# ezwelty/glimpse

Measured on NVIDIA B200. Metric: particle_updates_per_s, higher is better.
Workload: dtype f64

## Files before the change

### glimpse_b200/_lib.py

```python
from __future__ import annotations

import ctypes as C
import os

HERE = os.path.dirname(os.path.abspath(__file__))
LIB_PATH = os.path.join(HERE, "libglimpse_b200.so")

GB_MAX_OBS = 8
GB_ST_MESSAGES = {
    1: (ValueError, "Some particles are on non-visible viewshed cells"),
    2: (ValueError, "Some particles have missing (NaN) values"),
    3: (ValueError, "Some of the sampling coordinates are out of bounds"),
    4: (ValueError, "Some sampling points are outside box"),
    5: (IndexError, "Box extends beyond grid bounds"),
    6: (MemoryError, "Search window larger than the launch plan's surface capacity (template + 191 px per axis in mode='stream'; "
                     "the particle cloud has dispersed)"),
}
GB_OBS_OUT_OF_FRAME = 2
GB_ST_WINDOW_TOO_LARGE = 6
GB_WINDOW_MARGIN, GB_WINDOW_MARGIN_MAX = 191, 1000
GB_RNG_SUPPLIED, GB_RNG_PHILOX = 0, 1
GB_DRAW_WORDS, GB_DRAW_NORMALS, GB_DRAW_UNIFORM, GB_DRAW_UNIFORM_PARTICLE = 0, 1, 2, 3
GB_RESAMPLE = {"systematic": 0, "stratified": 1, "choice": 2, "residual": 3}
GB_MODE_STREAM = 1
# ... 77 lines not shown
        ("force_evolved", C.c_void_p), ("force_weights", C.c_void_p), ("dump_evolved", C.c_void_p),
        ("dump_uv", C.c_void_p), ("dump_box", C.c_void_p), ("dump_search", C.c_void_p), ("dump_sse", C.c_void_p),
        ("dump_sampled", C.c_void_p), ("dump_weights", C.c_void_p), ("dump_indices", C.c_void_p), ("dump_clocks", C.c_void_p), ("dump_cap", C.c_int64),
    ]


STRUCTS = (gb_camera, gb_image, gb_surface, gb_motion, gb_plan, gb_track_desc, gb_stage_io)

SIGNATURES = {
    "gb_version": (C.c_int, []),
    "gb_last_error": (C.c_char_p, []),
    "gb_struct_size": (C.c_int64, [C.c_int32]),
    "gb_sample_surface": (C.c_int, [C.c_void_p, C.c_int32, C.c_int32, C.c_int32, C.c_int32, C.c_void_p, C.c_int64, C.c_void_p, C.c_void_p, C.c_void_p]),
    "gb_kernel_timing": (C.c_int, [C.c_int32]),
    "gb_kernel_timing_read": (C.c_int, [C.POINTER(C.c_double), C.POINTER(C.c_int64), C.c_int32]),
    "gb_camera_from_vector": (C.c_int, [C.c_void_p, C.c_void_p, C.POINTER(gb_camera)]),
    "gb_project": (C.c_int, [C.POINTER(gb_camera), C.c_void_p, C.c_int64, C.c_void_p, C.c_void_p]),
    "gb_project_image": (C.c_int, [C.POINTER(gb_image), C.POINTER(gb_camera), C.c_int32, C.c_void_p, C.c_void_p]),
    "gb_viewshed_work_bytes": (C.c_int64, [C.c_int32, C.c_int32, C.c_int32]),
    "gb_viewshed": (C.c_int, [C.c_void_p, C.c_int32, C.c_int32, C.c_void_p, C.c_void_p, C.c_double, C.POINTER(C.c_double),
                              C.POINTER(C.c_double), C.c_int32, C.c_void_p, C.c_int64, C.c_void_p, C.c_void_p]),
    "gb_jpeg_info": (C.c_int, [C.c_char_p, C.c_int64, C.POINTER(C.c_int32), C.POINTER(C.c_int32), C.POINTER(C.c_int32)]),
    "gb_decode_jpeg": (C.c_int, [C.c_char_p, C.c_int64, C.c_int32, C.c_int32, C.c_int32, C.c_void_p, C.c_void_p]),
    "gb_unproject": (C.c_int, [C.POINTER(gb_camera), C.c_void_p, C.c_int64, C.c_int, C.c_void_p, C.c_void_p, C.c_void_p]),
    "gb_state_from_rows": (C.c_int, [C.c_void_p, C.c_int64, C.c_int64, C.c_void_p, C.c_void_p]),
    "gb_state_to_rows": (C.c_int, [C.c_void_p, C.c_int64, C.c_int64, C.c_void_p, C.c_void_p]),
    "gb_step_plan": (C.c_int, [C.c_int64, C.c_int32, C.c_int32, C.c_int64, C.c_int32, C.c_int32, C.c_int32, C.POINTER(gb_plan)]),
    "gb_step_plan_ex": (C.c_int, [C.c_int64, C.c_int32, C.c_int32, C.c_int64, C.c_int32, C.c_int32, C.c_int32, C.c_int32, C.POINTER(gb_plan)]),
    "gb_track": (C.c_int, [C.POINTER(gb_track_desc), C.c_void_p, C.POINTER(C.c_int64)]),
    "gb_track_step": (C.c_int, [C.POINTER(gb_track_desc), C.c_int32, C.POINTER(gb_stage_io), C.c_void_p]),
# ... 45 lines not shown
```

### glimpse_b200/csrc/camera.cuh

```cuda
#pragma once
#include "common.cuh"

namespace gb {

__device__ __forceinline__ void distort(const gb_camera& c, double x, double y, double& xd, double& yd) {
  const bool any_k = (c.k[0] != 0.0) | (c.k[1] != 0.0) | (c.k[2] != 0.0) | (c.k[3] != 0.0) | (c.k[4] != 0.0) |
                     (c.k[5] != 0.0);
  const bool any_p = (c.p[0] != 0.0) | (c.p[1] != 0.0);
  xd = x;
  yd = y;
  if (!any_k && !any_p) return;
  const double r2 = add(mul(x, x), mul(y, y));
  if (any_k) {
    double dr = 1.0;
    if (c.k[0] != 0.0) dr = add(dr, mul(c.k[0], r2));
    if (c.k[1] != 0.0) dr = add(dr, mul(mul(c.k[1], r2), r2));
    if (c.k[2] != 0.0) dr = add(dr, mul(mul(mul(c.k[2], r2), r2), r2));
    if ((c.k[3] != 0.0) | (c.k[4] != 0.0) | (c.k[5] != 0.0)) {
      double den = 1.0;
      if (c.k[3] != 0.0) den = add(den, mul(c.k[3], r2));
      if (c.k[4] != 0.0) den = add(den, mul(mul(c.k[4], r2), r2));
      if (c.k[5] != 0.0) den = add(den, mul(mul(mul(c.k[5], r2), r2), r2));
      dr = quo(dr, den);
    }
// ... 44 lines not shown
}

struct CamK {
  gb_camera c;
  int32_t any_k, any_p, has_den, pad_;
};

__host__ inline void camk_from(const gb_camera& c, CamK& out) {
  out.c = c;
  out.any_k = (c.k[0] != 0.0) || (c.k[1] != 0.0) || (c.k[2] != 0.0) || (c.k[3] != 0.0) || (c.k[4] != 0.0) || (c.k[5] != 0.0);
  out.has_den = (c.k[3] != 0.0) || (c.k[4] != 0.0) || (c.k[5] != 0.0);
  out.any_p = (c.p[0] != 0.0) || (c.p[1] != 0.0);
  out.pad_ = 0;
}

__device__ __forceinline__ void project_fast(const CamK& k, double px, double py, double pz, double& u, double& v) {
  const gb_camera& c = k.c;
  const double dx = px - c.xyz[0], dy = py - c.xyz[1];
  if (c.affine) {
    u = dx / c.f[0];
    v = dy / c.f[1];
    return;
  }
  double dz = pz - c.xyz[2];
  if (c.has_corr) dz = add(dz, quo(mul(c.corr_c1, add(mul(dx, dx), mul(dy, dy))), c.corr_c2));
  const double xc = fma(c.R[2], dz, fma(c.R[1], dy, c.R[0] * dx));
  const double yc = fma(c.R[5], dz, fma(c.R[4], dy, c.R[3] * dx));
  const double zc = fma(c.R[8], dz, fma(c.R[7], dy, c.R[6] * dx));
  double xd, yd;
  if (!k.any_k && !k.any_p) {
    const double iz = 1.0 / zc;
    xd = xc * iz;
    yd = yc * iz;
  } else {
    const double z2 = zc * zc, s = fma(xc, xc, yc * yc);
    const double s2 = s * s, z4 = z2 * z2;
    const double s3 = s2 * s, z6 = z4 * z2;
    const double sz4 = s * z4, s2z2 = s2 * z2;
    const double Nn = fma(c.k[2], s3, fma(c.k[1], s2z2, fma(c.k[0], sz4, z6)));
    const double Dd = k.has_den ? fma(c.k[5], s3, fma(c.k[4], s2z2, fma(c.k[3], sz4, z6))) : z6;
// ... 98 lines not shown
```

### glimpse_b200/csrc/glimpse_b200.cu

```cuda
#include <cuda.h>
#include <cuda_runtime.h>
#include <dlfcn.h>
#include <math.h>
#include <nvjpeg.h>
#include <stdio.h>
#include <stdlib.h>
#include <string.h>

#include <mutex>
#include <vector>

#include "camera.cuh"
#include "common.cuh"
#include "motion.cuh"
#include "tile.cuh"

#define GB_THREADS 512
#define GB_MAX_TEMPLATE 1024
#define GB_MAX_HIGHPASS 31

namespace gb {

static thread_local char g_error[512] = "";

// ... 75 lines not shown
  int64_t surf_bytes;
  int s_block, s_nblk;
  int tmpl_from_ev;
  int resample_method;
  int s2_budget;
  int s2_smem;
  int64_t p0, pb;
  int interp_rows, interp_cols;
};

struct NextParams {
  double tau, tau2;
  int spec_update, pad_;
  int img[GB_MAX_OBS];
  CamK cam[GB_MAX_OBS];
};

struct alignas(64) FrameMaps {
  CUtensorMap map[GB_MAX_OBS];
  int ok[GB_MAX_OBS];
};

__device__ __forceinline__ double* state_buffer(const StepParams& prm, int t) { return (t & 1) ? prm.state_b : prm.state_a; }

__device__ __forceinline__ int status_from_flags(uint32_t f) {
  if (f & GB_F_EVOLVE_OOB) return GB_ST_DEM_BOUNDS;
  if (f & GB_F_VIEW_OOB) return GB_ST_DEM_BOUNDS;
  if (f & GB_F_NOT_VISIBLE) return GB_ST_NOT_VISIBLE;
  if (f & GB_F_NAN) return GB_ST_NAN;
  if (f & GB_F_TEMPLATE) return GB_ST_TEMPLATE_BOUNDS;
  if (f & GB_F_WINDOW) return GB_ST_WINDOW_TOO_LARGE;
  if (f & GB_F_SAMPLE_OUTSIDE) return GB_ST_SAMPLE_OUTSIDE;
  if (f & GB_F_DEM_OOB) return GB_ST_DEM_BOUNDS;
  return GB_ST_OK;
}

__device__ __forceinline__ uint32_t test_particle(const StepParams& prm, const double (&s)[6]) {
  uint32_t f = 0;
  if (prm.viewshed >= 0) {
    bool oob;
    const double vis = surface_sample(prm.surfaces[prm.viewshed], s[0], s[1], 0, oob);
    if (oob) f |= GB_F_VIEW_OOB;
    else if (vis == 0.0) f |= GB_F_NOT_VISIBLE;
  }
  if (isnan(s[0]) | isnan(s[1]) | isnan(s[2]) | isnan(s[3]) | isnan(s[4]) | isnan(s[5])) f |= GB_F_NAN;
  return f;
}

template <bool COV>
struct Moments {
  static constexpr int NM = COV ? 28 : 13;
  double a[NM];
  __device__ __forceinline__ void clear() {
#pragma unroll
// ... 1002 lines not shown
    cudaEventRecord(next(), s);
  }
  void collect() {
    for (size_t i = 0; i < kind.size(); ++i) {
      float t = 0.f;
      if (cudaEventElapsedTime(&t, ev[2 * i], ev[2 * i + 1]) == cudaSuccess) {
        ms[kind[i]] += t;
        n[kind[i]] += 1;
      }
    }
    kind.clear();
    used = 0;
  }
};
static KernelTimer g_ktimer;

static int track_streaming(const gb_track_desc& d, cudaStream_t stream, int64_t* launches) {
  static std::once_flag attr_once[16];
  int dev = 0;
  GB_CUDA(cudaGetDevice(&dev));
  cudaError_t aerr = cudaSuccess;
  std::call_once(attr_once[dev & 15], [&]() {
    aerr = cudaFuncSetAttribute(k_s2_surface<false>, cudaFuncAttributeMaxDynamicSharedMemorySize, kSurfaceSmem);
    if (aerr == cudaSuccess) aerr = cudaFuncSetAttribute(k_s2_surface<true>, cudaFuncAttributeMaxDynamicSharedMemorySize, kSurfaceSmemLarge);
    if (aerr == cudaSuccess) aerr = cudaFuncSetAttribute(k_s4p_resample_propagate<true, true>, cudaFuncAttributeMaxDynamicSharedMemorySize, kS4pSmem);
    if (aerr == cudaSuccess) aerr = cudaFuncSetAttribute(k_s4p_resample_propagate<false, true>, cudaFuncAttributeMaxDynamicSharedMemorySize, kS4pSmem);
    if (aerr == cudaSuccess) aerr = cudaFuncSetAttribute(k_s4p_resample_propagate<true, false>, cudaFuncAttributeMaxDynamicSharedMemorySize, kS4pSmem);
    if (aerr == cudaSuccess) aerr = cudaFuncSetAttribute(k_s4p_resample_propagate<false, false>, cudaFuncAttributeMaxDynamicSharedMemorySize, kS4pSmem);
  });
  if (aerr != cudaSuccess) return fail(GB_E_CUDA, "stream kernel attributes: %s", cudaGetErrorString(aerr));
  if (d.plan.stream_block > GB_S4P_CAP || (d.plan.stream_block & 1)) return fail(GB_E_INVALID, "plan: stream_block must be even and <= 768%s");
  if (d.plan.stream_batch > 65535) return fail(GB_E_INVALID, "plan: stream_batch must be <= 65535%s");
  const bool cov = d.covariances != nullptr;
  const bool tangent = d.motion_kinds == 0 || (d.motion_kinds & ((1 << GB_MOTION_TANGENT_CARTESIAN) | (1 << GB_MOTION_TANGENT_CYLINDRICAL))) != 0;
  const int slots = d.plan.stream_slots;
  const int64_t batch = d.plan.stream_batch;
  const int64_t nbatch = (d.P + batch - 1) / batch;
  const int used = (int)(nbatch < slots ? nbatch : slots);
  StreamPool* pool = nullptr;
  int rc = get_pool(&pool);
  if (rc) return rc;
  std::lock_guard<std::mutex> guard(pool->busy);
  StepParams probe;
// ... 46 lines not shown
    if (launches) ++*launches;
  }
  bool have_activity = false;
  for (int t = 0; t < T; ++t) {
    if (!has_init[t] && !has_update[t] && !has_prop[t]) {
      have_activity = false;
      continue;
    }
    StepParams prm;
    fill_params(d, t, prm);
    NextParams nxt;
    memset(&nxt, 0, sizeof(nxt));
    for (int o = 0; o < GB_MAX_OBS; ++o) nxt.img[o] = -1;
    nxt.spec_update = has_init[t] ? 0 : 1;
    if (const char* e = getenv("GB_S4P_SPEC")) nxt.spec_update = nxt.spec_update && atoi(e) != 0;
    if (t + 1 < T) {
      StepParams pn;
      fill_params(d, t + 1, pn);
      nxt.tau = pn.tau;
      nxt.tau2 = pn.tau2;
      for (int o = 0; o < d.O; ++o) {
        nxt.img[o] = pn.img[o];
        nxt.cam[o] = pn.cam[o];
      }
    }
    FrameMaps fm;
    frame_maps(prm, fm);
    if (has_init[t] || has_tmpl[t]) {
      if ((rc = join_sides())) return rc;
      if ((rc = wait_images(stream, prm))) return rc;
      stream_bind(d, prm, t, 0, d.P);
      prm.tmpl_from_ev = 1;
      if (has_init[t]) {
        g_ktimer.begin(GB_K_INIT, stream);
        if ((rc = launch_init(prm, cov, stream))) return rc;
        g_ktimer.end(stream);
        if (launches) ++*launches;
      }
      if (has_tmpl[t]) {
        g_ktimer.begin(GB_K_TEMPLATE, stream);
// ... 31 lines not shown
          k_s2_surface<false><<<(unsigned)(pb * prm.O), GB_S2_THREADS, prm.s2_smem, ss>>>(prm, fm, prm.s2_budget);
        kt.end(ss);
        kt.begin(GB_K_WEIGHTS, ss);
        if (spline_is_hermite(prm.interp_cols, prm.interp_rows))
          k_s3_weights<false><<<dim3((unsigned)prm.s_nblk, (unsigned)pb), s3_threads(prm.s_block), 0, ss>>>(prm);
        else
          k_s3_weights<true><<<dim3((unsigned)prm.s_nblk, (unsigned)pb), s3_threads(prm.s_block), 0, ss>>>(prm);
        kt.end(ss);
        kt.begin(GB_K_PUBLISH, ss);
        k_s3b_publish<<<(unsigned)((pb + 7) / 8), 256, 0, ss>>>(prm);
        kt.end(ss);
      }
      kt.begin(GB_K_RESAMPLE_PROPAGATE, ss);
      {
        const dim3 grid((unsigned)prm.s_nblk, (unsigned)pb);
        if (cov && tangent)
          k_s4p_resample_propagate<true, true><<<grid, GB_S4P_THREADS, kS4pSmem, ss>>>(prm, nxt);
        else if (cov)
          k_s4p_resample_propagate<true, false><<<grid, GB_S4P_THREADS, kS4pSmem, ss>>>(prm, nxt);
        else if (tangent)
          k_s4p_resample_propagate<false, true><<<grid, GB_S4P_THREADS, kS4pSmem, ss>>>(prm, nxt);
        else
          k_s4p_resample_propagate<false, false><<<grid, GB_S4P_THREADS, kS4pSmem, ss>>>(prm, nxt);
      }
      kt.end(ss);
      kt.begin(GB_K_FINALIZE, ss);
      if (cov)
        k_s5p_finalize<true><<<(unsigned)((pb + 3) / 4), 128, 0, ss>>>(prm);
      else
        k_s5p_finalize<false><<<(unsigned)((pb + 3) / 4), 128, 0, ss>>>(prm);
      kt.end(ss);
      GB_CUDA(cudaGetLastError());
      if (launches) *launches += (has_update[t] ? 5 : 2) + (need_activity ? 1 : 0);
    }
  }
  if ((rc = join_sides())) return rc;
  if (g_ktimer.on) {
    GB_CUDA(cudaStreamSynchronize(stream));
// ... 118 lines not shown
    case 5: return sizeof(gb_track_desc);
    case 6: return sizeof(gb_stage_io);
    default: return -1;
  }
}

int gb_kernel_timing(int32_t enable) {
  std::lock_guard<std::mutex> guard(gb::g_ktimer.mu);
  gb::g_ktimer.on = enable != 0;
  gb::g_ktimer.kind.clear();
  gb::g_ktimer.used = 0;
  for (int k = 0; k < gb::GB_K_KINDS; ++k) {
    gb::g_ktimer.ms[k] = 0.0;
    gb::g_ktimer.n[k] = 0;
  }
  return GB_OK;
}

int gb_kernel_timing_read(double* ms, int64_t* launches, int32_t n) {
  if (!ms || !launches || n < 0) return gb::fail(GB_E_INVALID, "null argument%s");
  std::lock_guard<std::mutex> guard(gb::g_ktimer.mu);
  for (int k = 0; k < n; ++k) {
    ms[k] = k < gb::GB_K_KINDS ? gb::g_ktimer.ms[k] : 0.0;
    launches[k] = k < gb::GB_K_KINDS ? gb::g_ktimer.n[k] : 0;
  }
  return GB_OK;
}

int gb_camera_from_vector(const double* v, const double* corr, gb_camera* out) {
  if (!v || !out) return fail(GB_E_INVALID, "null argument%s");
// ... 434 lines not shown
```

### glimpse_b200/csrc/motion.cuh

```cuda
#pragma once
#include "common.cuh"

namespace gb {

struct Philox {
  uint32_t key0, key1;
  __device__ __forceinline__ static void round(uint32_t (&c)[4], uint32_t k0, uint32_t k1) {
    const uint32_t hi0 = __umulhi(0xD2511F53u, c[0]), lo0 = 0xD2511F53u * c[0];
    const uint32_t hi1 = __umulhi(0xCD9E8D57u, c[2]), lo1 = 0xCD9E8D57u * c[2];
    const uint32_t n0 = hi1 ^ c[1] ^ k0, n2 = hi0 ^ c[3] ^ k1;
    c[0] = n0;
    c[1] = lo1;
    c[2] = n2;
    c[3] = lo0;
  }
  __device__ __forceinline__ void generate(uint32_t c0, uint32_t c1, uint32_t c2, uint32_t c3, uint32_t (&out)[4]) const {
    uint32_t c[4] = {c0, c1, c2, c3};
    uint32_t k0 = key0, k1 = key1;
#pragma unroll
    for (int i = 0; i < 10; ++i) {
      round(c, k0, k1);
      k0 += 0x9E3779B9u;
      k1 += 0xBB67AE85u;
    }
    out[0] = c[0];
    out[1] = c[1];
    out[2] = c[2];
    out[3] = c[3];
  }
};

__device__ __forceinline__ void philox_normals3(uint64_t seed, uint64_t point, uint32_t time, uint32_t particle,
                                                uint32_t stream, double& z0, double& z1, double& z2, int need = 3) {
  Philox g{(uint32_t)seed, (uint32_t)(seed >> 32)};
  uint32_t r[4];
  g.generate(particle, time, (uint32_t)point, ((uint32_t)(point >> 32) << 8) | stream, r);
  const float two_neg32 = 2.3283064365386963e-10f;
  z0 = z1 = z2 = 0.0;
  if (need & 1) {
    const float u0 = ((float)r[0] + 0.5f) * two_neg32;
    const float a0 = fminf(fmaxf(u0, 1.0e-10f), 1.0f);
    const float e0 = fmaxf(-2.0f * __logf(a0), 1.0e-30f);
    const float rad0 = e0 * rsqrtf(e0);
    float s0, c0;
    __sincosf(6.283185307179586f * ((float)(r[1] >> 8) * 5.9604644775390625e-08f), &s0, &c0);
    z0 = (double)(rad0 * c0);
    z1 = (double)(rad0 * s0);
  }
  if (need & 2) {
    const float u1 = ((float)r[2] + 0.5f) * two_neg32;
    const float a1 = fminf(fmaxf(u1, 1.0e-10f), 1.0f);
    const float e1 = fmaxf(-2.0f * __logf(a1), 1.0e-30f);
    const float rad1 = e1 * rsqrtf(e1);
    z2 = (double)(rad1 * __cosf(6.283185307179586f * ((float)(r[3] >> 8) * 5.9604644775390625e-08f)));
  }
}

__device__ __forceinline__ bool motion_is_tangent(const gb_motion& m) { return m.kind >= GB_MOTION_TANGENT_CARTESIAN; }
__device__ __forceinline__ bool motion_is_cylindrical(const gb_motion& m) {
  return m.kind == GB_MOTION_CYLINDRICAL || m.kind == GB_MOTION_TANGENT_CYLINDRICAL;
}

__device__ __forceinline__ int evolve_needs(const gb_motion& m) {
  const double third = motion_is_tangent(m) ? m.slope_sigma : m.a_sigma[2];
  return ((m.a_sigma[0] != 0.0 || m.a_sigma[1] != 0.0) ? 1 : 0) | (third != 0.0 ? 2 : 0);
}

__device__ __forceinline__ double philox_uniform(uint64_t seed, uint64_t point, uint32_t time) {
  Philox g{(uint32_t)seed, (uint32_t)(seed >> 32)};
// ... 108 lines not shown
```

### glimpse_b200/csrc/stream.cuh

```cuda
#pragma once

#define GB_SBLOCK_THREADS 256

#define GB_ACT_ACTIVE 1
#define GB_ACT_SURFACE_LL 2
#define GB_ACT_NO_MOTION_LL 8
__device__ __forceinline__ bool stream_point_active(const StepParams& prm, int64_t p) {
  return (prm.s_act[p] & GB_ACT_ACTIVE) != 0;
}

__global__ void k_s0_reset(const __grid_constant__ StepParams prm) {
  const int64_t lo5 = prm.p0 * prm.O * 5, n = prm.pb * prm.O * 5;
  for (int64_t i = blockIdx.x * (int64_t)blockDim.x + threadIdx.x; i < n; i += (int64_t)gridDim.x * blockDim.x)
    prm.s_ibox[lo5 + i] = (i % 5 == 4) ? 0 : 0x7fffffff;
  for (int64_t i = prm.p0 + blockIdx.x * (int64_t)blockDim.x + threadIdx.x; i < prm.p0 + prm.pb; i += (int64_t)gridDim.x * blockDim.x) {
    prm.s_pflags[i] = 0;
    const bool active = prm.status[i] == 0 && prm.t > prm.first[i] && prm.t <= prm.last[i];
    const gb_surface& sg = prm.surfaces[prm.motion[i].dem_sigma];
    const bool tangent = prm.motion[i].kind >= GB_MOTION_TANGENT_CARTESIAN;
    const bool sll = !tangent && !(sg.z == nullptr && sg.value == 0.0);
    prm.s_act[i] = (uint8_t)((active ? GB_ACT_ACTIVE : 0) | (sll ? GB_ACT_SURFACE_LL : 0) | (tangent ? GB_ACT_NO_MOTION_LL : 0));
  }
}

// ... 1037 lines not shown
  }
}

#ifndef GB_S4P_THREADS
#define GB_S4P_THREADS 192
#endif
#ifndef GB_S4P_CAP
#define GB_S4P_CAP 768
#endif
#ifndef GB_S4P_MINB
#define GB_S4P_MINB 4
#endif
#define GB_S4P_PPT ((GB_S4P_CAP + GB_S4P_THREADS - 1) / GB_S4P_THREADS)
constexpr int kS4pSmem = GB_S4P_CAP * 64;
static_assert(GB_S4P_THREADS >= 134, "k_s4p's prologue spreads its scalar loads over the first 134 threads");

__device__ __forceinline__ void s4p_project_child(const CamK& cam, const double (&s)[6], double* uv, int64_t N, int j, double hw,
                                                  double hh, int (&e)[5]) {
  double u, v;
  project_fast(cam, s[0], s[1], s[2], u, v);
  uv[j] = u;
  uv[N + j] = v;
  e[0] = __double2int_rd(u - hw);
  e[1] = __double2int_rd(v - hh);
  e[2] = -__double2int_ru(u + hw);
  e[3] = -__double2int_ru(v + hh);
  e[4] = (isnan(u) | isnan(v)) ? -1 : 0;
}

template <bool COV, bool TAN>
__global__ void __launch_bounds__(GB_S4P_THREADS, GB_S4P_MINB) k_s4p_resample_propagate(const __grid_constant__ StepParams prm,
                                                                                   const __grid_constant__ NextParams nxt) {
  constexpr int NM = Moments<COV>::NM, KP = COV ? 32 : 16, PPT = GB_S4P_PPT, CAP = GB_S4P_CAP, NW = GB_S4P_THREADS / 32, TH = GB_S4P_THREADS;
  extern __shared__ __align__(128) unsigned char s4p_raw[];
  double* s_st = reinterpret_cast<double*>(s4p_raw);
  double* s_w = s_st + 6 * CAP;
  int* s_end = reinterpret_cast<int*>(s_w + CAP);
  int* s_par = s_end + CAP;
  __shared__ __align__(8) uint64_t s_bar[2];
  __shared__ double s_warp[NW];
  __shared__ double s_red[NW][KP];
  __shared__ int s_wmax[NW];
  __shared__ int s_j0;
  __shared__ gb_motion s_motion;
  __shared__ int s_box[GB_MAX_OBS][5];
  __shared__ unsigned s_or;
  __shared__ double s_pre6[6];
  __shared__ double s_refv[6];
// ... 38 lines not shown
  if ((!update && !propagate) || failed_at_t != 0) {
    if (spec && tid == 0) {
      mbar_wait(&s_bar[0], 0);
      mbar_wait(&s_bar[1], 0);
    }
    return;
  }
  const double* src6 = (update ? prm.s_ev : state_buffer(prm, t)) + p * 6 * (int64_t)N + base;
  const bool bulk = n_here > 0 && ((N | n_here) & 1) == 0 && ((reinterpret_cast<uintptr_t>(src6) | reinterpret_cast<uintptr_t>(wsrc)) & 15) == 0;
  if (tid < (int)(sizeof(gb_motion) / 4)) reinterpret_cast<uint32_t*>(&s_motion)[tid] = motion_word;
  if (propagate && tid < GB_MAX_OBS * 5) s_box[tid / 5][tid % 5] = (tid % 5 == 4) ? 0 : 0x7fffffff;
  if (tid >= 64 && tid < 70) s_refv[tid - 64] = ref_word;
  if (tid >= 96 && tid < 96 + O) s_mask[tid - 96] = mask_byte;
  if (tid >= 128 && tid < 134) s_pre6[tid - 128] = ref_word;
  __syncthreads();
  if (bulk) {
    if (tid == 0 && !spec) {
      const uint32_t row = (uint32_t)n_here * 8u;
      if (update) {
        mbar_expect_tx(&s_bar[0], row);
        bulk_load(s_w, wsrc, row, &s_bar[0]);
      }
      mbar_expect_tx(&s_bar[1], 6u * row);
#pragma unroll
      for (int c = 0; c < 6; ++c) bulk_load(s_st + c * CAP, src6 + c * (int64_t)N, row, &s_bar[1]);
    }
  } else {
    for (int i = tid; i < n_here; i += TH) {
      if (update) s_w[i] = wsrc[i];
#pragma unroll
      for (int c = 0; c < 6; ++c) s_st[c * CAP + i] = src6[c * (int64_t)N + i];
    }
  }
  int J0, J1;
  if (update) {
    const double prefix = s_pre6[0], next_prefix = s_pre6[1], total = s_pre6[2], inv_total = s_pre6[3], u01 = s_pre6[4],
                 inv_n = s_pre6[5];
    const bool stratified = prm.resample_method == GB_RESAMPLE_STRATIFIED;
    const double dN = (double)N;
    if (bulk) mbar_wait(&s_bar[0], 0);
    else __syncthreads();
    const int k0 = PPT * tid;
    double w[PPT];
    double tsum = 0.0;
#pragma unroll
    for (int q = 0; q < PPT; ++q) {
      tsum += (k0 + q < n_here) ? s_w[k0 + q] : 0.0;
      w[q] = tsum;
    }
    const double off = block_exclusive_offset<NW>(tsum, s_warp);
#pragma unroll
    for (int q = 0; q < PPT; ++q) {
      const int k = k0 + q;
// ... 2 lines not shown
        const double cn = c >= total ? 1.0 : c * inv_total;
        s_end[k] = stratified ? count_positions_le_stratified(cn, stratified_draws(prm, p, t), inv_n, N) : count_positions_le_fast(cn, u01, inv_n, N, dN);
      }
    }
    if (tid == 0) {
      const double c0 = prefix >= total ? 1.0 : prefix * inv_total;
      s_j0 = b == 0 ? 0 : stratified ? count_positions_le_stratified(c0, stratified_draws(prm, p, t), inv_n, N) : count_positions_le_fast(c0, u01, inv_n, N, dN);
    }
    __syncthreads();
    J0 = s_j0;
    J1 = n_here > 0 ? s_end[n_here - 1] : J0;
  } else {
    J0 = base;
    J1 = base + n_here;
  }
  if (bulk) mbar_wait(&s_bar[1], 0);
  else if (!update) __syncthreads();
  if (update) {
    double ref[6];
#pragma unroll
    for (int c = 0; c < 6; ++c) ref[c] = s_refv[c];
    Moments<COV> mom;
    mom.clear();
#pragma unroll
    for (int q = 0; q < PPT; ++q) {
      const int k = tid + q * TH;
      if (k < n_here) {
        const int cnt = s_end[k] - (k > 0 ? s_end[k - 1] : J0);
        if (cnt > 0) {
          double s[6];
#pragma unroll
          for (int c = 0; c < 6; ++c) s[c] = s_st[c * CAP + k];
// ... 1 lines not shown
        }
      }
    }
    double r[KP];
#pragma unroll
    for (int k = 0; k < KP; ++k) r[k] = k < NM ? mom.a[k] : 0.0;
    warp_reduce_transpose<KP>(r, lane);
    if (KP == 32 || (lane & 1) == 0) s_red[warp][transposed_index<KP>(lane)] = r[0];
    __syncthreads();
    if (tid < NM) {
      double x = s_red[0][tid];
      for (int wv = 1; wv < NW; ++wv) x += s_red[wv][tid];
      prm.s_pm[(p * prm.s_nblk + b) * 28 + tid] = x;
    }
  }
  const bool last_time = !propagate;
  double* sout = state_buffer(prm, t) + p * 6 * (int64_t)N;
  double* evn = prm.s_ev_next + p * 6 * (int64_t)N;
  double* wst = prm.weight_state ? prm.weight_state + (int64_t)p * N : nullptr;
  double* outp = (update && prm.out_particles) ? prm.out_particles + ((int64_t)p * prm.T + t) * N * 6 : nullptr;
  double* outw = (update && prm.out_weights) ? prm.out_weights + ((int64_t)p * prm.T + t) * N : nullptr;
  const int s_idx = (t + 1) - prm.first[p] - 1;
  const double* zn = (propagate && prm.step_normals) ? prm.step_normals + (((int64_t)p * prm.S + s_idx) * N) * 3 : nullptr;
  const double hw = (double)prm.tile_w * 0.5, hh = (double)prm.tile_h * 0.5;
  uint32_t flags = 0;
  const int need = propagate ? evolve_needs(s_motion) : 0;
  int ibx[2][5];
#pragma unroll
  for (int o = 0; o < 2; ++o) {
    ibx[o][0] = ibx[o][1] = ibx[o][2] = ibx[o][3] = 0x7fffffff;
    ibx[o][4] = 0;
  }
  unsigned obs_on = 0;
  if (propagate)
    for (int o = 0; o < O; ++o)
      if (nxt.img[o] >= 0 && s_mask[o]) obs_on |= 1u << o;
  int carry = 0;
  for (int Jc = J0; Jc < J1; Jc += CAP) {
    const int nch = min(CAP, J1 - Jc);
    if (update) {
      for (int i = tid; i < nch; i += TH) s_par[i] = 0;
      __syncthreads();
#pragma unroll
      for (int q = 0; q < PPT; ++q) {
        const int k = tid + q * TH;
        if (k < n_here) {
          const int st = k > 0 ? s_end[k - 1] : J0, en = s_end[k];
          if (en > st && st >= Jc && st - Jc < nch) s_par[st - Jc] = k;
        }
      }
      __syncthreads();
      int v[PPT], run = 0;
#pragma unroll
      for (int q = 0; q < PPT; ++q) {
// ... 15 lines not shown
        const int x = s_wmax[k];
        if (k < warp) pre = max(pre, x);
        all = max(all, x);
      }
      int excl = __shfl_up_sync(0xffffffffu, incl, 1);
      if (lane == 0) excl = 0;
      pre = max(pre, excl);
#pragma unroll
      for (int q = 0; q < PPT; ++q) {
        const int i = PPT * tid + q;
        if (i < nch) s_par[i] = max(pre, v[q]);
      }
      carry = all;
      __syncthreads();
    }
    for (int j = Jc + tid; j < Jc + nch; j += TH) {
      const int lo = update ? s_par[j - Jc] : j - base;
      double s[6];
#pragma unroll
      for (int c = 0; c < 6; ++c) s[c] = s_st[c * CAP + lo];
      if (update) {
        const double wj = s_w[lo];
        if (last_time) {
#pragma unroll
          for (int c = 0; c < 6; ++c) __stcs(&sout[c * (int64_t)N + j], s[c]);
          if (prm.final_weights && p == prm.P - 1) prm.final_weights[j] = wj;
        }
        if (wst) wst[j] = wj;
        if (outp) {
#pragma unroll
          for (int c = 0; c < 6; ++c) outp[(int64_t)j * 6 + c] = s[c];
        }
        if (outw) outw[j] = wj;
      }
      if (propagate) {
        double z0, z1, z2;
        if (prm.rng_mode == GB_RNG_SUPPLIED) {
          z0 = zn[3 * (int64_t)j];
          z1 = zn[3 * (int64_t)j + 1];
          z2 = zn[3 * (int64_t)j + 2];
        } else {
          philox_normals3(prm.seed, (uint64_t)(p + prm.point_offset), (uint32_t)(t + 1), (uint32_t)j, 2u, z0, z1, z2, need);
        }
        evolve_particle<TAN>(s_motion, prm.surfaces, nxt.tau, nxt.tau2, z0, z1, z2, s, flags);
        flags |= test_particle(prm, s);
#pragma unroll
        for (int c = 0; c < 6; ++c) evn[c * (int64_t)N + j] = s[c];
#pragma unroll
        for (int o = 0; o < 2; ++o) {
          if (o >= O) break;
          if (!(obs_on >> o & 1)) continue;
          const int64_t po = p * O + o;
          int e[5];
          s4p_project_child(nxt.cam[o], s, prm.s_uv + po * 2 * (int64_t)N, N, j, hw, hh, e);
#pragma unroll
          for (int k = 0; k < 5; ++k) ibx[o][k] = min(ibx[o][k], e[k]);
        }
        for (int o = 2; o < O; ++o) {
          if (!(obs_on >> o & 1)) continue;
          const int64_t po = p * O + o;
          int e[5];
          s4p_project_child(nxt.cam[o], s, prm.s_uv + po * 2 * (int64_t)N, N, j, hw, hh, e);
#pragma unroll
          for (int k = 0; k < 5; ++k) atomicMin(&s_box[o][k], e[k]);
        }
      }
    }
    if (update && Jc + CAP < J1) __syncthreads();
  }
  if (propagate) {
#pragma unroll
    for (int o = 0; o < 2; ++o) {
      if (o >= O) break;
      int mine = 0x7fffffff;
#pragma unroll
      for (int k = 0; k < 5; ++k) {
        const int x = __reduce_min_sync(0xffffffffu, ibx[o][k]);
        if (lane == k) mine = x;
      }
      if (lane < 5) atomicMin(&s_box[o][lane], mine);
    }
    const int any = (int)block_or(flags, &s_or);
    if (any && tid == 0) atomicOr(&prm.s_pflags_next[p], any);
    if (tid < O * 5) {
      const int o = tid / 5, k = tid - o * 5;
      const int64_t po = p * O + o;
      if (obs_on >> o & 1) atomicMin(&prm.s_ibox[po * 5 + k], s_box[o][k]);
    }
  }
}

template <bool COV>
__global__ void k_s5p_finalize(const __grid_constant__ StepParams prm) {
  const int64_t p = prm.p0 + ((blockIdx.x * (int64_t)blockDim.x + threadIdx.x) >> 5);
  const int lane = threadIdx.x & 31;
  if (p >= prm.p0 + prm.pb) return;
  const int act = prm.s_act[p];
  const int t = prm.t;
  const int f = prm.s_pflags[p];
  if (lane == 0) prm.s_pflags[p] = 0;
  if (!(act & GB_ACT_ACTIVE)) {
    if (lane == 0) {
      bool alive = prm.status[p] == 0;
      if (f && alive && t > prm.first[p] && t <= prm.last[p]) {
// ... 40 lines not shown
```

### include/glimpse_b200.h

```cpp
#ifndef GLIMPSE_B200_H
#define GLIMPSE_B200_H

#include <stdint.h>

#ifdef __cplusplus
extern "C" {
#endif

#define GB_VERSION 1

#define GB_OK 0
#define GB_E_INVALID (-1)
#define GB_E_CUDA (-2)
#define GB_E_RESOURCE (-3)

#define GB_ST_OK 0
#define GB_ST_NOT_VISIBLE 1
#define GB_ST_NAN 2
#define GB_ST_DEM_BOUNDS 3
#define GB_ST_SAMPLE_OUTSIDE 4
#define GB_ST_TEMPLATE_BOUNDS 5
#define GB_ST_WINDOW_TOO_LARGE 6

#define GB_OBS_USED 0
// ... 64 lines not shown
int gb_version(void);
const char* gb_last_error(void);
int64_t gb_struct_size(int32_t which);

#define GB_KERNEL_ACTIVITY 0
#define GB_KERNEL_SURFACE 1
#define GB_KERNEL_WEIGHTS 2
#define GB_KERNEL_RESAMPLE_PROPAGATE 3
#define GB_KERNEL_FINALIZE 4
#define GB_KERNEL_INIT 5
#define GB_KERNEL_TEMPLATE 6
#define GB_KERNEL_PUBLISH 7
#define GB_KERNEL_KINDS 8
int gb_kernel_timing(int32_t enable);
int gb_kernel_timing_read(double* ms, int64_t* launches, int32_t n);
int gb_camera_from_vector(const double* vec20_host, const double* corr_host, gb_camera* out_host);

int gb_project(const gb_camera* cam_host, const double* xyz, int64_t n, double* uv, void* stream);
int gb_unproject(const gb_camera* cam_host, const double* uv, int64_t n, int directions, const double* depth,
                 double* xyz, void* stream);

int gb_project_image(const gb_image* src_host, const gb_camera* dst_cam_host, int32_t method, void* out, void* stream);

int gb_jpeg_info(const uint8_t* jpeg_host, int64_t nbytes, int32_t* width, int32_t* height, int32_t* nchan);
int gb_decode_jpeg(const uint8_t* jpeg_host, int64_t nbytes, int32_t width, int32_t height, int32_t nchan, uint8_t* out, void* stream);

int64_t gb_viewshed_work_bytes(int32_t nx, int32_t ny, int32_t max_rings);
int gb_viewshed(const double* z, int32_t nx, int32_t ny, const double* x_centres, const double* y_centres, double cell,
                const double* origin_host, const double* corr_host, int32_t max_rings, void* work, int64_t work_bytes,
                uint8_t* visible, void* stream);
// ... 145 lines not shown
```

Measured before the change: 18.58 billion.

## Add lean specialization of resample-propagate kernel with precomputed Philox keys

Adds a LEAN template variant of the stream resample/propagate kernel, used for the common configuration: Philox RNG, systematic resampling, no viewshed, one observer, no output dumps, and a plain pinhole camera. The variant compiles out the branches for those options, and it precomputes the Philox key schedule on the host. It also hoists the per-point first Philox round so each particle only runs the remaining rounds. The change also adds optional clock64 instrumentation and a launch counter. It trades extra template instantiations, and so larger binary and compile time, for fewer instructions and less register pressure in the hot loop.

```diff
diff --git a/glimpse_b200/_lib.py b/glimpse_b200/_lib.py
--- a/glimpse_b200/_lib.py
+++ b/glimpse_b200/_lib.py
@@ -115,6 +115,7 @@
     "gb_sample_surface": (C.c_int, [C.c_void_p, C.c_int32, C.c_int32, C.c_int32, C.c_int32, C.c_void_p, C.c_int64, C.c_void_p, C.c_void_p, C.c_void_p]),
     "gb_kernel_timing": (C.c_int, [C.c_int32]),
     "gb_kernel_timing_read": (C.c_int, [C.POINTER(C.c_double), C.POINTER(C.c_int64), C.c_int32]),
+    "gb_s4p_lean_launches": (C.c_int, [C.POINTER(C.c_int64)]),
     "gb_camera_from_vector": (C.c_int, [C.c_void_p, C.c_void_p, C.POINTER(gb_camera)]),
     "gb_project": (C.c_int, [C.POINTER(gb_camera), C.c_void_p, C.c_int64, C.c_void_p, C.c_void_p]),
     "gb_project_image": (C.c_int, [C.POINTER(gb_image), C.POINTER(gb_camera), C.c_int32, C.c_void_p, C.c_void_p]),
diff --git a/glimpse_b200/csrc/camera.cuh b/glimpse_b200/csrc/camera.cuh
--- a/glimpse_b200/csrc/camera.cuh
+++ b/glimpse_b200/csrc/camera.cuh
@@ -82,16 +82,17 @@
   out.pad_ = 0;
 }
 
+template <bool PLAIN = false>
 __device__ __forceinline__ void project_fast(const CamK& k, double px, double py, double pz, double& u, double& v) {
   const gb_camera& c = k.c;
   const double dx = px - c.xyz[0], dy = py - c.xyz[1];
-  if (c.affine) {
+  if (!PLAIN && c.affine) {
     u = dx / c.f[0];
     v = dy / c.f[1];
     return;
   }
   double dz = pz - c.xyz[2];
-  if (c.has_corr) dz = add(dz, quo(mul(c.corr_c1, add(mul(dx, dx), mul(dy, dy))), c.corr_c2));
+  if (!PLAIN && c.has_corr) dz = add(dz, quo(mul(c.corr_c1, add(mul(dx, dx), mul(dy, dy))), c.corr_c2));
   const double xc = fma(c.R[2], dz, fma(c.R[1], dy, c.R[0] * dx));
   const double yc = fma(c.R[5], dz, fma(c.R[4], dy, c.R[3] * dx));
   const double zc = fma(c.R[8], dz, fma(c.R[7], dy, c.R[6] * dx));
diff --git a/glimpse_b200/csrc/glimpse_b200.cu b/glimpse_b200/csrc/glimpse_b200.cu
--- a/glimpse_b200/csrc/glimpse_b200.cu
+++ b/glimpse_b200/csrc/glimpse_b200.cu
@@ -7,6 +7,7 @@
 #include <stdlib.h>
 #include <string.h>
 
+#include <atomic>
 #include <mutex>
 #include <vector>
 
@@ -113,6 +114,8 @@
   int spec_update, pad_;
   int img[GB_MAX_OBS];
   CamK cam[GB_MAX_OBS];
+  uint32_t philox_key[20];
+  long long* clocks;
 };
 
 struct alignas(64) FrameMaps {
@@ -134,9 +137,10 @@
   return GB_ST_OK;
 }
 
+template <bool VIEWSHED = true>
 __device__ __forceinline__ uint32_t test_particle(const StepParams& prm, const double (&s)[6]) {
   uint32_t f = 0;
-  if (prm.viewshed >= 0) {
+  if (VIEWSHED && prm.viewshed >= 0) {
     bool oob;
     const double vis = surface_sample(prm.surfaces[prm.viewshed], s[0], s[1], 0, oob);
     if (oob) f |= GB_F_VIEW_OOB;
@@ -1169,6 +1173,15 @@
   }
 };
 static KernelTimer g_ktimer;
+static std::atomic<int64_t> g_s4p_lean_launches{0};
+
+#if defined(GB_S4P_CLOCKS) && GB_S4P_CLOCKS
+static long long* g_s4p_clocks = nullptr;
+extern "C" int gb_s4p_clocks(int64_t* buffer) {
+  g_s4p_clocks = reinterpret_cast<long long*>(buffer);
+  return GB_OK;
+}
+#endif
 
 static int track_streaming(const gb_track_desc& d, cudaStream_t stream, int64_t* launches) {
   static std::once_flag attr_once[16];
@@ -1178,10 +1191,12 @@
   std::call_once(attr_once[dev & 15], [&]() {
     aerr = cudaFuncSetAttribute(k_s2_surface<false>, cudaFuncAttributeMaxDynamicSharedMemorySize, kSurfaceSmem);
     if (aerr == cudaSuccess) aerr = cudaFuncSetAttribute(k_s2_surface<true>, cudaFuncAttributeMaxDynamicSharedMemorySize, kSurfaceSmemLarge);
-    if (aerr == cudaSuccess) aerr = cudaFuncSetAttribute(k_s4p_resample_propagate<true, true>, cudaFuncAttributeMaxDynamicSharedMemorySize, kS4pSmem);
-    if (aerr == cudaSuccess) aerr = cudaFuncSetAttribute(k_s4p_resample_propagate<false, true>, cudaFuncAttributeMaxDynamicSharedMemorySize, kS4pSmem);
-    if (aerr == cudaSuccess) aerr = cudaFuncSetAttribute(k_s4p_resample_propagate<true, false>, cudaFuncAttributeMaxDynamicSharedMemorySize, kS4pSmem);
-    if (aerr == cudaSuccess) aerr = cudaFuncSetAttribute(k_s4p_resample_propagate<false, false>, cudaFuncAttributeMaxDynamicSharedMemorySize, kS4pSmem);
+    if (aerr == cudaSuccess) aerr = cudaFuncSetAttribute(k_s4p_resample_propagate<true, true, false>, cudaFuncAttributeMaxDynamicSharedMemorySize, kS4pSmem);
+    if (aerr == cudaSuccess) aerr = cudaFuncSetAttribute(k_s4p_resample_propagate<false, true, false>, cudaFuncAttributeMaxDynamicSharedMemorySize, kS4pSmem);
+    if (aerr == cudaSuccess) aerr = cudaFuncSetAttribute(k_s4p_resample_propagate<true, false, false>, cudaFuncAttributeMaxDynamicSharedMemorySize, kS4pSmem);
+    if (aerr == cudaSuccess) aerr = cudaFuncSetAttribute(k_s4p_resample_propagate<false, false, false>, cudaFuncAttributeMaxDynamicSharedMemorySize, kS4pSmem);
+    if (aerr == cudaSuccess) aerr = cudaFuncSetAttribute(k_s4p_resample_propagate<true, false, true>, cudaFuncAttributeMaxDynamicSharedMemorySize, kS4pSmem);
+    if (aerr == cudaSuccess) aerr = cudaFuncSetAttribute(k_s4p_resample_propagate<false, false, true>, cudaFuncAttributeMaxDynamicSharedMemorySize, kS4pSmem);
   });
   if (aerr != cudaSuccess) return fail(GB_E_CUDA, "stream kernel attributes: %s", cudaGetErrorString(aerr));
   if (d.plan.stream_block > GB_S4P_CAP || (d.plan.stream_block & 1)) return fail(GB_E_INVALID, "plan: stream_block must be even and <= 768%s");
@@ -1258,6 +1273,10 @@
     for (int o = 0; o < GB_MAX_OBS; ++o) nxt.img[o] = -1;
     nxt.spec_update = has_init[t] ? 0 : 1;
     if (const char* e = getenv("GB_S4P_SPEC")) nxt.spec_update = nxt.spec_update && atoi(e) != 0;
+    philox_key_schedule(d.seed, nxt.philox_key);
+#if defined(GB_S4P_CLOCKS) && GB_S4P_CLOCKS
+    nxt.clocks = g_s4p_clocks;
+#endif
     if (t + 1 < T) {
       StepParams pn;
       fill_params(d, t + 1, pn);
@@ -1268,6 +1287,10 @@
         nxt.cam[o] = pn.cam[o];
       }
     }
+    bool lean = GB_S4P_LEAN && !tangent && prm.rng_mode == GB_RNG_PHILOX && prm.resample_method == GB_RESAMPLE_SYSTEMATIC && prm.viewshed < 0 &&
+                !prm.out_particles && !prm.out_weights && !prm.weight_state && d.O == 1;
+    for (int o = 0; o < d.O; ++o)
+      if (nxt.img[o] >= 0 && (nxt.cam[o].c.affine || nxt.cam[o].c.has_corr)) lean = false;
     FrameMaps fm;
     frame_maps(prm, fm);
     if (has_init[t] || has_tmpl[t]) {
@@ -1329,14 +1352,19 @@
       kt.begin(GB_K_RESAMPLE_PROPAGATE, ss);
       {
         const dim3 grid((unsigned)prm.s_nblk, (unsigned)pb);
-        if (cov && tangent)
-          k_s4p_resample_propagate<true, true><<<grid, GB_S4P_THREADS, kS4pSmem, ss>>>(prm, nxt);
+        if (lean) ++g_s4p_lean_launches;
+        if (lean && cov)
+          k_s4p_resample_propagate<true, false, true><<<grid, GB_S4P_THREADS, kS4pSmem, ss>>>(prm, nxt);
+        else if (lean)
+          k_s4p_resample_propagate<false, false, true><<<grid, GB_S4P_THREADS, kS4pSmem, ss>>>(prm, nxt);
+        else if (cov && tangent)
+          k_s4p_resample_propagate<true, true, false><<<grid, GB_S4P_THREADS, kS4pSmem, ss>>>(prm, nxt);
         else if (cov)
-          k_s4p_resample_propagate<true, false><<<grid, GB_S4P_THREADS, kS4pSmem, ss>>>(prm, nxt);
+          k_s4p_resample_propagate<true, false, false><<<grid, GB_S4P_THREADS, kS4pSmem, ss>>>(prm, nxt);
         else if (tangent)
-          k_s4p_resample_propagate<false, true><<<grid, GB_S4P_THREADS, kS4pSmem, ss>>>(prm, nxt);
+          k_s4p_resample_propagate<false, true, false><<<grid, GB_S4P_THREADS, kS4pSmem, ss>>>(prm, nxt);
         else
-          k_s4p_resample_propagate<false, false><<<grid, GB_S4P_THREADS, kS4pSmem, ss>>>(prm, nxt);
+          k_s4p_resample_propagate<false, false, false><<<grid, GB_S4P_THREADS, kS4pSmem, ss>>>(prm, nxt);
       }
       kt.end(ss);
       kt.begin(GB_K_FINALIZE, ss);
@@ -1485,6 +1513,12 @@
     gb::g_ktimer.ms[k] = 0.0;
     gb::g_ktimer.n[k] = 0;
   }
+  return GB_OK;
+}
+
+int gb_s4p_lean_launches(int64_t* out) {
+  if (!out) return fail(GB_E_INVALID, "null output%s");
+  *out = g_s4p_lean_launches.load();
   return GB_OK;
 }
 
diff --git a/glimpse_b200/csrc/motion.cuh b/glimpse_b200/csrc/motion.cuh
--- a/glimpse_b200/csrc/motion.cuh
+++ b/glimpse_b200/csrc/motion.cuh
@@ -30,11 +30,7 @@
   }
 };
 
-__device__ __forceinline__ void philox_normals3(uint64_t seed, uint64_t point, uint32_t time, uint32_t particle,
-                                                uint32_t stream, double& z0, double& z1, double& z2, int need = 3) {
-  Philox g{(uint32_t)seed, (uint32_t)(seed >> 32)};
-  uint32_t r[4];
-  g.generate(particle, time, (uint32_t)point, ((uint32_t)(point >> 32) << 8) | stream, r);
+__device__ __forceinline__ void box_muller3(const uint32_t (&r)[4], int need, double& z0, double& z1, double& z2) {
   const float two_neg32 = 2.3283064365386963e-10f;
   z0 = z1 = z2 = 0.0;
   if (need & 1) {
@@ -53,6 +49,40 @@
     const float e1 = fmaxf(-2.0f * __logf(a1), 1.0e-30f);
     const float rad1 = e1 * rsqrtf(e1);
     z2 = (double)(rad1 * __cosf(6.283185307179586f * ((float)(r[3] >> 8) * 5.9604644775390625e-08f)));
+  }
+}
+
+__device__ __forceinline__ void philox_normals3(uint64_t seed, uint64_t point, uint32_t time, uint32_t particle,
+                                                uint32_t stream, double& z0, double& z1, double& z2, int need = 3) {
+  Philox g{(uint32_t)seed, (uint32_t)(seed >> 32)};
+  uint32_t r[4];
+  g.generate(particle, time, (uint32_t)point, ((uint32_t)(point >> 32) << 8) | stream, r);
+  box_muller3(r, need, z0, z1, z2);
+}
+
+struct PhiloxPoint {
+  uint32_t n0, lo1, x3;
+};
+__device__ __forceinline__ PhiloxPoint philox_point_round(const uint32_t* key, uint64_t point, uint32_t time, uint32_t stream) {
+  const uint32_t c2 = (uint32_t)point, c3 = ((uint32_t)(point >> 32) << 8) | stream;
+  return PhiloxPoint{__umulhi(0xCD9E8D57u, c2) ^ time ^ key[0], 0xCD9E8D57u * c2, c3 ^ key[1]};
+}
+__device__ __forceinline__ void philox_particle_words(const uint32_t* key, const PhiloxPoint& h, uint32_t particle, uint32_t (&c)[4]) {
+  c[0] = h.n0;
+  c[1] = h.lo1;
+  c[2] = __umulhi(0xD2511F53u, particle) ^ h.x3;
+  c[3] = 0xD2511F53u * particle;
+#pragma unroll
+  for (int i = 1; i < 10; ++i) Philox::round(c, key[2 * i], key[2 * i + 1]);
+}
+
+__host__ inline void philox_key_schedule(uint64_t seed, uint32_t (&key)[20]) {
+  uint32_t k0 = (uint32_t)seed, k1 = (uint32_t)(seed >> 32);
+  for (int i = 0; i < 10; ++i) {
+    key[2 * i] = k0;
+    key[2 * i + 1] = k1;
+    k0 += 0x9E3779B9u;
+    k1 += 0xBB67AE85u;
   }
 }
 
diff --git a/glimpse_b200/csrc/stream.cuh b/glimpse_b200/csrc/stream.cuh
--- a/glimpse_b200/csrc/stream.cuh
+++ b/glimpse_b200/csrc/stream.cuh
@@ -1075,11 +1075,22 @@
 #define GB_S4P_PPT ((GB_S4P_CAP + GB_S4P_THREADS - 1) / GB_S4P_THREADS)
 constexpr int kS4pSmem = GB_S4P_CAP * 64;
 static_assert(GB_S4P_THREADS >= 134, "k_s4p's prologue spreads its scalar loads over the first 134 threads");
-
+#ifndef GB_S4P_LEAN
+#define GB_S4P_LEAN 1
+#endif
+
+#if defined(GB_S4P_CLOCKS) && GB_S4P_CLOCKS
+#define S4P_CLK(k) \
+  if (tid == 0) s_ck[k] = clock64()
+#else
+#define S4P_CLK(k)
+#endif
+
+template <bool PLAIN>
 __device__ __forceinline__ void s4p_project_child(const CamK& cam, const double (&s)[6], double* uv, int64_t N, int j, double hw,
                                                   double hh, int (&e)[5]) {
   double u, v;
-  project_fast(cam, s[0], s[1], s[2], u, v);
+  project_fast<PLAIN>(cam, s[0], s[1], s[2], u, v);
   uv[j] = u;
   uv[N + j] = v;
   e[0] = __double2int_rd(u - hw);
@@ -1089,10 +1100,17 @@
   e[4] = (isnan(u) | isnan(v)) ? -1 : 0;
 }
 
-template <bool COV, bool TAN>
+template <bool COV, bool TAN, bool LEAN>
 __global__ void __launch_bounds__(GB_S4P_THREADS, GB_S4P_MINB) k_s4p_resample_propagate(const __grid_constant__ StepParams prm,
                                                                                    const __grid_constant__ NextParams nxt) {
   constexpr int NM = Moments<COV>::NM, KP = COV ? 32 : 16, PPT = GB_S4P_PPT, CAP = GB_S4P_CAP, NW = GB_S4P_THREADS / 32, TH = GB_S4P_THREADS;
+#if defined(GB_S4P_CLOCKS) && GB_S4P_CLOCKS
+  __shared__ long long s_ck[10];
+  if (threadIdx.x == 0) {
+    s_ck[0] = clock64();
+    s_ck[8] = s_ck[9] = 0;
+  }
+#endif
   extern __shared__ __align__(128) unsigned char s4p_raw[];
   double* s_st = reinterpret_cast<double*>(s4p_raw);
   double* s_w = s_st + 6 * CAP;
@@ -1161,6 +1179,7 @@
   if (tid >= 96 && tid < 96 + O) s_mask[tid - 96] = mask_byte;
   if (tid >= 128 && tid < 134) s_pre6[tid - 128] = ref_word;
   __syncthreads();
+  S4P_CLK(1);
   if (bulk) {
     if (tid == 0 && !spec) {
       const uint32_t row = (uint32_t)n_here * 8u;
@@ -1183,7 +1202,7 @@
   if (update) {
     const double prefix = s_pre6[0], next_prefix = s_pre6[1], total = s_pre6[2], inv_total = s_pre6[3], u01 = s_pre6[4],
                  inv_n = s_pre6[5];
-    const bool stratified = prm.resample_method == GB_RESAMPLE_STRATIFIED;
+    const bool stratified = !LEAN && prm.resample_method == GB_RESAMPLE_STRATIFIED;
     const double dN = (double)N;
     if (bulk) mbar_wait(&s_bar[0], 0);
     else __syncthreads();
@@ -1216,8 +1235,10 @@
     J0 = base;
     J1 = base + n_here;
   }
+  S4P_CLK(2);
   if (bulk) mbar_wait(&s_bar[1], 0);
   else if (!update) __syncthreads();
+  S4P_CLK(3);
   if (update) {
     double ref[6];
 #pragma unroll
@@ -1249,12 +1270,13 @@
       prm.s_pm[(p * prm.s_nblk + b) * 28 + tid] = x;
     }
   }
+  S4P_CLK(4);
   const bool last_time = !propagate;
   double* sout = state_buffer(prm, t) + p * 6 * (int64_t)N;
   double* evn = prm.s_ev_next + p * 6 * (int64_t)N;
-  double* wst = prm.weight_state ? prm.weight_state + (int64_t)p * N : nullptr;
-  double* outp = (update && prm.out_particles) ? prm.out_particles + ((int64_t)p * prm.T + t) * N * 6 : nullptr;
-  double* outw = (update && prm.out_weights) ? prm.out_weights + ((int64_t)p * prm.T + t) * N : nullptr;
+  double* wst = (!LEAN && prm.weight_state) ? prm.weight_state + (int64_t)p * N : nullptr;
+  double* outp = (!LEAN && update && prm.out_particles) ? prm.out_particles + ((int64_t)p * prm.T + t) * N * 6 : nullptr;
+  double* outw = (!LEAN && update && prm.out_weights) ? prm.out_weights + ((int64_t)p * prm.T + t) * N : nullptr;
   const int s_idx = (t + 1) - prm.first[p] - 1;
   const double* zn = (propagate && prm.step_normals) ? prm.step_normals + (((int64_t)p * prm.S + s_idx) * N) * 3 : nullptr;
   const double hw = (double)prm.tile_w * 0.5, hh = (double)prm.tile_h * 0.5;
@@ -1270,9 +1292,11 @@
   if (propagate)
     for (int o = 0; o < O; ++o)
       if (nxt.img[o] >= 0 && s_mask[o]) obs_on |= 1u << o;
+  const PhiloxPoint php = philox_point_round(nxt.philox_key, (uint64_t)(p + prm.point_offset), (uint32_t)(t + 1), 2u);
   int carry = 0;
   for (int Jc = J0; Jc < J1; Jc += CAP) {
     const int nch = min(CAP, J1 - Jc);
+    S4P_CLK(5);
     if (update) {
       for (int i = tid; i < nch; i += TH) s_par[i] = 0;
       __syncthreads();
@@ -1318,6 +1342,7 @@
       carry = all;
       __syncthreads();
     }
+    S4P_CLK(6);
     for (int j = Jc + tid; j < Jc + nch; j += TH) {
       const int lo = update ? s_par[j - Jc] : j - base;
       double s[6];
@@ -1339,37 +1364,48 @@
       }
       if (propagate) {
         double z0, z1, z2;
-        if (prm.rng_mode == GB_RNG_SUPPLIED) {
+        if (!LEAN && prm.rng_mode == GB_RNG_SUPPLIED) {
           z0 = zn[3 * (int64_t)j];
           z1 = zn[3 * (int64_t)j + 1];
           z2 = zn[3 * (int64_t)j + 2];
+        } else if (LEAN) {
+          uint32_t r[4];
+          philox_particle_words(nxt.philox_key, php, (uint32_t)j, r);
+          box_muller3(r, need, z0, z1, z2);
         } else {
           philox_normals3(prm.seed, (uint64_t)(p + prm.point_offset), (uint32_t)(t + 1), (uint32_t)j, 2u, z0, z1, z2, need);
         }
         evolve_particle<TAN>(s_motion, prm.surfaces, nxt.tau, nxt.tau2, z0, z1, z2, s, flags);
-        flags |= test_particle(prm, s);
+        flags |= test_particle<!LEAN>(prm, s);
 #pragma unroll
         for (int c = 0; c < 6; ++c) evn[c * (int64_t)N + j] = s[c];
 #pragma unroll
-        for (int o = 0; o < 2; ++o) {
+        for (int o = 0; o < (LEAN ? 1 : 2); ++o) {
           if (o >= O) break;
           if (!(obs_on >> o & 1)) continue;
           const int64_t po = p * O + o;
           int e[5];
-          s4p_project_child(nxt.cam[o], s, prm.s_uv + po * 2 * (int64_t)N, N, j, hw, hh, e);
+          s4p_project_child<LEAN>(nxt.cam[o], s, prm.s_uv + po * 2 * (int64_t)N, N, j, hw, hh, e);
 #pragma unroll
           for (int k = 0; k < 5; ++k) ibx[o][k] = min(ibx[o][k], e[k]);
         }
-        for (int o = 2; o < O; ++o) {
+        for (int o = 2; o < (LEAN ? 0 : O); ++o) {
           if (!(obs_on >> o & 1)) continue;
           const int64_t po = p * O + o;
           int e[5];
-          s4p_project_child(nxt.cam[o], s, prm.s_uv + po * 2 * (int64_t)N, N, j, hw, hh, e);
+          s4p_project_child<false>(nxt.cam[o], s, prm.s_uv + po * 2 * (int64_t)N, N, j, hw, hh, e);
 #pragma unroll
           for (int k = 0; k < 5; ++k) atomicMin(&s_box[o][k], e[k]);
         }
       }
     }
+#if defined(GB_S4P_CLOCKS) && GB_S4P_CLOCKS
+    if (tid == 0) {
+      const long long now = clock64();
+      s_ck[8] += s_ck[6] - s_ck[5];
+      s_ck[9] += now - s_ck[6];
+    }
+#endif
     if (update && Jc + CAP < J1) __syncthreads();
   }
   if (propagate) {
@@ -1392,6 +1428,17 @@
       if (obs_on >> o & 1) atomicMin(&prm.s_ibox[po * 5 + k], s_box[o][k]);
     }
   }
+#if defined(GB_S4P_CLOCKS) && GB_S4P_CLOCKS
+  if (tid == 0 && b == 0 && nxt.clocks) {
+    const long long end = clock64();
+    long long* out = nxt.clocks + p * 16;
+    for (int k = 0; k < 4; ++k) out[k] += s_ck[k + 1] - s_ck[k];
+    out[4] += s_ck[8];
+    out[5] += s_ck[9];
+    out[6] += end - s_ck[4] - s_ck[8] - s_ck[9];
+    out[15] += 1;
+  }
+#endif
 }
 
 template <bool COV>
diff --git a/include/glimpse_b200.h b/include/glimpse_b200.h
--- a/include/glimpse_b200.h
+++ b/include/glimpse_b200.h
@@ -102,6 +102,7 @@
 #define GB_KERNEL_KINDS 8
 int gb_kernel_timing(int32_t enable);
 int gb_kernel_timing_read(double* ms, int64_t* launches, int32_t n);
+int gb_s4p_lean_launches(int64_t* out_host);
 int gb_camera_from_vector(const double* vec20_host, const double* corr_host, gb_camera* out_host);
 
 int gb_project(const gb_camera* cam_host, const double* xyz, int64_t n, double* uv, void* stream);
```

After: 19.73 billion, median of 6. 6.2% higher.
